# learningmatter-mit/surface-sampling

Hardware: AMD Instinct MI355X
Metric: MC energy-evaluations/sec (SrTiO3(001) ~250-atom slabs, 3-model PaiNN ensemble E+F incl. neighbor list) (higher is better)
Workload: dtype f32 via fp16x2-split MFMA (3 products), fp32 accumulate; neighbor decisions f64; 1 GPU; SrTiO3(001) PaiNN x3, 256 batched independent chains per GPU (BASELINE configs[3]), 248-272 atoms/chain; chains_per_gpu=256, atoms_per_gpu=66503, edges_per_gpu=2747786, slots_per_gpu=2836316, models=3, streams_per_gpu=2, parallelism=one GPU, no collective

## Files before the change

### surface-sampling_amd/csrc/api_batch.hip

```cpp
#include <cmath>
#include <cstdio>

#include "cell_dev.h"
#include "ewald_dev.h"

using namespace vssr;

extern "C" {

int vssr_batch_upload(vssr_handle *h, int32_t n_cfg, const int32_t *n_atoms, const int32_t *Z, const double *pos,
                      const double *cell, const uint8_t *pbc) {
    if (int rc = check_kind(h, KINDS_EVAL, __func__)) return rc;
    if (n_cfg < 1 || !n_atoms || !Z || !pos || !cell || !pbc) return set_err(h, VSSR_E_BADARG, "null or empty batch");
    VSSR_HIP(h, hipSetDevice(h->device));
    VSSR_HIP(h, hipStreamSynchronize(h->stream));
    h->batch_valid = false;
    h->ran = false;
    h->md_vel_valid = false;
    std::vector<int> start(n_cfg + 1, 0);
    for (int b = 0; b < n_cfg; ++b) {
        if (n_atoms[b] < 1) return set_err(h, VSSR_E_BADARG, "configuration %d has %d atoms", b, n_atoms[b]);
        if ((int64_t)start[b] + n_atoms[b] > 2000000000LL) return set_err(h, VSSR_E_BADARG, "batch too large");
        start[b + 1] = start[b] + n_atoms[b];
    }
// ... 571 lines not shown
    int l;
    if ((l = layer_of("phi")) >= 0) {
        if (l == 0 && h->l0_used)
            return set_err(h, VSSR_E_STATE, "phi0 is not materialised (layer-0 species factorisation is active)");
        src = sv.phi[l]; per_atom = F3;
    }
    else if ((l = layer_of("s_msg")) >= 0) { src = sv.s_msg[l]; per_atom = F; }
    else if ((l = layer_of("v_msg")) >= 0) { src = sv.v_msg[l]; per_atom = F3; }
    else if ((l = layer_of("s_upd")) >= 0) { src = sv.s_in[l + 1]; per_atom = F; }
    else if ((l = layer_of("v_upd")) >= 0) {
        if (l == h->num_conv - 1 && !h->debug_keep)
            return set_err(h, VSSR_E_STATE, "v_upd of the last block is not materialised (nothing consumes it; create the handle with VSSR_DEBUG_KEEP=1)");
        src = sv.v_in[l + 1]; per_atom = F3;
    }
    else if (nm == "e_atom") { src = sv.e_atom; per_atom = 1; }
    else if (nm == "sbar_msg0") { src = sv.sbar_msg_l0; per_atom = F; }
    else if (nm == "vbar_msg0") { src = sv.vbar_msg; per_atom = F3; }
    else return set_err(h, VSSR_E_BADARG, "unknown intermediate '%s'", name);
    size_t n = N * per_atom;
    *n_out = (int64_t)n;
    if (!dst) return VSSR_OK;
    if ((int64_t)n > cap) return set_err(h, VSSR_E_BADARG, "buffer too small for '%s'", name);
    VSSR_HIP(h, hipMemcpy(dst, src + (size_t)model * n, n * sizeof(float), hipMemcpyDeviceToHost));
    return VSSR_OK;
}

}
```

### surface-sampling_amd/csrc/api_painn.hip

```cpp
#include <cmath>

#include "vssr_internal.h"

namespace vssr {

static void transpose(const float *src, int rows, int cols, float *dst) {
    for (int r = 0; r < rows; ++r)
        for (int c = 0; c < cols; ++c) dst[(size_t)c * rows + r] = src[(size_t)r * cols + c];
}

static int upload_weights(vssr_handle *h, const vssr_painn_config *cfg) {
    const int M = cfg->n_models, L = cfg->num_conv, R = cfg->n_rbf, H = cfg->readout_hidden, NE = cfg->n_embed;
    const size_t per_layer = (size_t)F * F + F + (size_t)F3 * F + F3 + (size_t)F3 * R + F3 + 2 * (size_t)F * F +
                             (size_t)F * 2 * F + F + (size_t)F3 * F + F3;
    const size_t blob_len = (size_t)NE * F + L * per_layer + (size_t)H * F + H + H + 1;
    if (cfg->weights_len != blob_len)
        return set_err(h, VSSR_E_BADARG, "weights_len %llu does not match the layout (%zu floats)",
                       (unsigned long long)cfg->weights_len, blob_len);
    const size_t t_per_layer = (size_t)F * F + (size_t)F * F3 + 2 * (size_t)F * F + (size_t)2 * F * F + (size_t)F * F3;
    const size_t img_len = blob_len + L * t_per_layer + (size_t)F * H;
    std::vector<float> img(img_len * M);
    std::vector<ModelW> table(M);
    if (h->weights.ensure(img.size() * sizeof(float)))
        return set_err(h, VSSR_E_NOMEM, "weights: out of device memory");
// ... 115 lines not shown
        if (h->d_l0A.ensure(A16.size() * sizeof(unsigned)) || h->d_l0At.ensure(At16.size() * sizeof(unsigned)))
            return set_err(h, VSSR_E_NOMEM, "layer-0 tables");
        VSSR_HIP(h, hipMemcpy(h->d_l0A.p, A16.data(), A16.size() * sizeof(unsigned), hipMemcpyHostToDevice));
        VSSR_HIP(h, hipMemcpy(h->d_l0At.p, At16.data(), At16.size() * sizeof(unsigned), hipMemcpyHostToDevice));
    }
    if (h->model_table.ensure(sizeof(ModelW) * M)) return set_err(h, VSSR_E_NOMEM, "model table");
    VSSR_HIP(h, hipMemcpy(h->model_table.p, table.data(), sizeof(ModelW) * M, hipMemcpyHostToDevice));
    return VSSR_OK;
}

static void read_env_knobs(vssr_handle *h) {
    if (const char *e = getenv("VSSR_PAINN_PATH")) h->painn_general = h->painn_general || strcmp(e, "general") == 0;
    if (const char *e = getenv("VSSR_EDGE_IMPL")) h->edge_impl = (strcmp(e, "gather") == 0) ? 0 : 1;
    if (const char *e = getenv("VSSR_L0_FACTORISE")) h->l0_enabled = atoi(e);
    if (h->painn_general) h->l0_enabled = 0;
    if (const char *e = getenv("VSSR_UPD_SAVE")) h->upd_save = atoi(e);
    if (const char *e = getenv("VSSR_DEBUG_KEEP")) h->debug_keep = atoi(e);
    if (const char *e = getenv("VSSR_EDGE_FS16_MAX")) h->fs16_max_atoms = atoi(e);
    if (const char *e = getenv("VSSR_EDGE_FS8_MAX")) h->fs8_max_atoms = atoi(e);
    if (const char *e = getenv("VSSR_EDGE_BWD_MPASS")) h->bwd_multi_pass = atoi(e);
    if (const char *e = getenv("VSSR_EDGE_SUB_CHUNK")) { const int c = atoi(e); if (c >= 8) { h->sub_chunk_fwd = c; h->sub_chunk_bwd = c; } }
    if (const char *e = getenv("VSSR_EDGE_FWD_2PASS")) { const int w = atoi(e); h->fwd_two_pass = (w == 8 || w == 16) ? w : w ? 16 : 0; }
    if (const char *e = getenv("VSSR_EDGE_FWD_GRID")) h->edge_fwd_grid = max(atoi(e), 0);
}

}

using namespace vssr;

extern "C" {
// ... 47 lines not shown
```

### surface-sampling_amd/csrc/mfma16.h

```cpp
#ifndef VSSR_MFMA16_H
#define VSSR_MFMA16_H
#include "vssr_internal.h"

namespace vssr {

typedef float f32x4 __attribute__((ext_vector_type(4)));
typedef float f32x2 __attribute__((ext_vector_type(2)));
typedef unsigned u32x4 __attribute__((ext_vector_type(4)));
typedef unsigned u32x2 __attribute__((ext_vector_type(2)));
typedef _Float16 f16x8 __attribute__((ext_vector_type(8)));
typedef _Float16 f16x2 __attribute__((ext_vector_type(2)));

constexpr int TA = 32;
constexpr int NW = 8;
constexpr int NTHREADS = 64 * NW;
constexpr int PADH = 8;

#ifndef VSSR_FAST_SIGMOID
#define VSSR_FAST_SIGMOID 1
#endif
__device__ __forceinline__ float sigm(float x) {
#if VSSR_FAST_SIGMOID && defined(__HIP_DEVICE_COMPILE__)
    constexpr float C_HI = -1.44269502162933349609375f;
    constexpr float C_LO = -1.9259629911266175e-08f;
// ... 179 lines not shown
    return *reinterpret_cast<gptr>(reinterpret_cast<uintptr_t>(p));
#else
    return *reinterpret_cast<const f32x4 *>(p);
#endif
}

__device__ __forceinline__ float gload1f(const float *p) {
#if defined(__HIP_DEVICE_COMPILE__)
    typedef const float __attribute__((address_space(1))) *gptr;
    return *reinterpret_cast<gptr>(reinterpret_cast<uintptr_t>(p));
#else
    return *p;
#endif
}

}
#endif
```

### surface-sampling_amd/csrc/painn.hip

```cpp
#include "vssr_internal.h"

namespace vssr {

constexpr int T = NODE_TILE;
constexpr int RB = 21;
constexpr int ECHUNK = 16;
constexpr float PI_F = 3.14159265358979323846f;

__device__ inline float sigmoidf_(float x) { return 1.f / (1.f + expf(-x)); }
__device__ inline float swishf_(float x) { return x * sigmoidf_(x); }
__device__ inline float dswishf_(float x) {
    float sg = sigmoidf_(x);
    return sg * fmaf(x, 1.f - sg, 1.f);
}

__global__ void __launch_bounds__(128) k_embed(int N, const int *__restrict__ Z, const ModelW *__restrict__ MW,
                                               float *__restrict__ s0, float *__restrict__ v0) {
    int i = blockIdx.x, m = blockIdx.y, f = threadIdx.x;
    const ModelW &W = MW[m];
    size_t a = (size_t)m * N + i;
    s0[a * F + f] = W.embed[(size_t)Z[i] * F + f];
    v0[(a * 3 + 0) * F + f] = 0.f;
    v0[(a * 3 + 1) * F + f] = 0.f;
    v0[(a * 3 + 2) * F + f] = 0.f;
// ... 598 lines not shown
                launch_edge_fwd_mfma(st, cls, N, cls_list[cls], h->n_class[cls], M, l, h->max_class_atoms[cls], MW, G, counters,
                                     (int)(h->slot_cap - 1), sv.s_in[l], sv.v_in[l], sv.phi[l], sv.s_msg[l], sv.v_msg[l],
                                     (cls == EDGE_CLASS_FS4 && h->fwd_two_pass) ? h->d_bundle_sub.as<int4>() : (const int4 *)nullptr,
                                     h->fwd_two_pass, h->sub_chunk_fwd ? h->sub_chunk_fwd : sub_chunk_max(h->fwd_two_pass), h->edge_fwd_grid);
            if (n_gather)
                hipLaunchKernelGGL(k_edge_fwd<false>, g_atom, blk, 0, st, N, l, MW, G, counters, h->cutoff, h->excl_vol,
                                   h->excl_sigma, h->excl_power, sv.s_in[l], sv.v_in[l], sv.phi[l], sv.s_msg[l],
                                   sv.v_msg[l], (int)EDGE_BCLASS_GATHER);
        }
        P.end(st);
        update_fwd(l);
    }
    const bool fused = readout_mfma_supported(H);
    const bool want_forces = (want & VSSR_WANT_FORCES) != 0;
    const float *e_excl = h->excl_vol ? sv.e_excl : (const float *)nullptr;
    if (!(fused && want_forces)) {
        P.begin(KC_READOUT, st);
        if (fused) launch_readout_mfma(st, N, M, av, MW, sv.s_in[L], e_excl, sv.e_atom);
        else
            hipLaunchKernelGGL(k_readout, g_tile, blk, 0, st, N, H, av, MW, sv.s_in[L], sv.e_excl, h->excl_vol, sv.e_atom,
                               sv.sbar);
        P.end(st);
    }

    if (want_forces) {
        float *sb_buf[2] = {sv.sbar_msg, sv.sbar};
        for (int l = L - 1; l >= 0; --l) {
            float *sbar_msg_l = fused ? sb_buf[(L - 1 - l) & 1] : sv.sbar_msg;
            const float *sbar_msg_up = sb_buf[(L - l) & 1];
            P.begin(KC_UPDATE_BWD, st);
            if (!fused)
                launch_update_bwd_mfma(st, N, M, l, 0, (int)(l == L - 1), av, MW, sv.s_msg[l], sv.v_msg[l], sv.sbar, sv.vbar,
                                       nullptr, nullptr, nullptr, nullptr, sbar_msg_l, sv.vbar_msg, nullptr, nullptr);
            else if (l == L - 1 && fuse_last)
                launch_update_bwd_mfma(st, N, M, l, 3, 1, av, MW, sv.s_msg[l], sv.v_msg[l], nullptr, sv.vbar, nullptr, nullptr,
                                       e_excl, sv.e_atom, sbar_msg_l, sv.vbar_msg, sv.s_in[L], nullptr);
            else if (l == L - 1)
                launch_update_bwd_mfma(st, N, M, l, 1, 1, av, MW, sv.s_msg[l], sv.v_msg[l], nullptr, sv.vbar, sv.s_in[L], nullptr,
                                       e_excl, sv.e_atom, sbar_msg_l, sv.vbar_msg, nullptr, save_of(l));
            else
                launch_update_bwd_mfma(st, N, M, l, 2, 0, av, MW, sv.s_msg[l], sv.v_msg[l], sbar_msg_up, sv.vbar, sv.s_in[l + 1],
                                       sv.phibar, nullptr, nullptr, sbar_msg_l, sv.vbar_msg, nullptr, save_of(l));
            P.end(st);
            sv.sbar_msg_l0 = sbar_msg_l;
            P.begin((l == 0 && l0_fact) ? KC_L0_BWD : KC_EDGE_BWD, st);
            int accumulate = (l != L - 1);
            if (l == 0 && l0_fact) {
                rc = l0_run_reverse(h, G, (int)(L == 1), (int)partial, sbar_msg_l, sv.vbar_msg, sv.gbar);
                if (rc) return rc;
            } else if (l == 0)
                hipLaunchKernelGGL(k_edge_bwd<true>, g_atom, blk, 0, st, N, l, accumulate, MW, G, counters,
                                   h->cutoff, h->excl_vol, h->excl_sigma, h->excl_power, sv.v_in[l], sv.phi[l],
                                   sbar_msg_l, sv.vbar_msg, sv.phibar, sv.vbar, sv.gbar,
                                   (long long)h->slot_cap, -1, (int)partial);
            else {
                for (int cls = 0; cls < EDGE_MFMA_BCLASSES; ++cls)
                    launch_edge_bwd_mfma(st, cls, N, bcls_list[cls], h->n_bclass[cls], M, l, h->max_bclass_atoms[cls], MW, G, counters,
                                         (int)(h->slot_cap - 1), sv.v_in[l], sv.phi[l], sbar_msg_l, sv.vbar_msg, sv.phibar, sv.vbar,
                                         h->d_gpart.as<float>(), (long long)h->slot_cap, n_groups, (L - 1 - l) * per_set,
                                         cls == EDGE_BCLASS_FS16P ? h->d_bundle_subb.as<int4>() : (const int4 *)nullptr,
                                         h->sub_chunk_bwd ? h->sub_chunk_bwd : sub_chunk_max_bwd());
                if (n_gather)
                    hipLaunchKernelGGL(k_edge_bwd<false>, g_atom, blk, 0, st, N, l, accumulate, MW, G, counters,
// ... 11 lines not shown
    }
    P.begin(KC_FINALIZE, st);
    if (want_forces && partial) {
        const int uni = h->active_mask ? 0 : h->n_bclass[EDGE_BCLASS_FS16] + h->n_bclass[EDGE_BCLASS_FS16P] == h->n_cfg ? 8 : h->n_bclass[EDGE_BCLASS_FS8] == h->n_cfg ? 16
                        : h->n_bclass[EDGE_BCLASS_FS4] == h->n_cfg ? 32 : 0;
        const dim3 grid = uni ? dim3((unsigned)((h->slot_cap + 255) / 256), 1) : dim3(h->n_cfg, 12);
        hipLaunchKernelGGL(k_reduce_gpart, grid, dim3(256), 0, st, M, n_groups, layer_sets, G, counters, h->d_gpart.as<float>(),
                           sv.gbar, (long long)h->slot_cap, uni);
    }
    painn_finalize(h, G, want);
    P.end(st);
    VSSR_HIP(h, hipGetLastError());
    return VSSR_OK;
}

void painn_finalize(vssr_handle *h, const GraphView &G, uint32_t want) {
    const int N = h->n_atoms, M = h->n_models;
    hipStream_t st = h->stream;
    if (want & VSSR_WANT_FORCES)
        hipLaunchKernelGGL(k_finalize_forces, dim3((N + 3) / 4), dim3(256), 0, st, N, M, G, h->d_counters.as<int>(), h->sv.gbar,
                           (long long)h->slot_cap, h->units_per_ev, h->d_forces.as<float>(), h->d_forces_std.as<float>());
    hipLaunchKernelGGL(k_finalize_energy, dim3(h->n_cfg), dim3(256), 0, st, N, M, h->active_mask, G.cfg_start, h->d_Z.as<int>(),
                       h->sv.e_atom, h->units_per_ev, h->has_offset ? h->offset_per_z.as<double>() : (const double *)nullptr,
                       h->offset_const, h->d_energy.as<float>(), h->d_energy_std.as<float>(), h->d_energy_models.as<float>(),
                       h->d_energy64.as<double>(), h->d_e_atoms.as<float>(), h->d_sat.as<unsigned>(), h->d_sat_out.as<unsigned>());
}

int painn_stress(vssr_handle *h) {
    if (h->d_stress.ensure(sizeof(double) * 12 * (size_t)h->n_cfg)) return set_err(h, VSSR_E_DEVICE, "out of device memory (stress)");
    double *out = h->d_stress.as<double>();
// ... 8 lines not shown
```

### surface-sampling_amd/csrc/painn_l0.hip

```cpp
#include "mfma16.h"

namespace vssr {

constexpr int KP = 24;
constexpr int TBLK = 4 * KP;

template <int NZ>
__global__ void __launch_bounds__(96)
k_l0_accum(GraphView G, const int *__restrict__ counters, float *__restrict__ T) {
    constexpr int nz = NZ;
    if (counters[2] || !G.act.atom(blockIdx.x)) return;
    const int i = blockIdx.x, comp = threadIdx.x / KP, kap = threadIdx.x % KP;
    float acc[NZ];
#pragma unroll
    for (int z = 0; z < NZ; ++z) acc[z] = 0.f;
    auto erec_c = [&](int idx) -> float4 {
#if defined(__HIP_DEVICE_COMPILE__)
        typedef const f32x4 __attribute__((address_space(4))) *cp;
        const f32x4 v = reinterpret_cast<cp>(reinterpret_cast<uintptr_t>(G.erec))[idx];
        return make_float4(v.x, v.y, v.z, v.w);
#else
        return G.erec[idx];
#endif
    };
// ... 17 lines not shown
            r[u] = G.rho[(size_t)(e + u) * KP + kap];
            zi[u] = (zw >> (8 * u)) & 255;
        }
#pragma unroll
        for (int u = 0; u < 4; ++u) {
            const float uu = comp == 0 ? 1.f : comp == 1 ? er[u].x : comp == 2 ? er[u].y : er[u].z;
            const float val = r[u] * uu;
#pragma unroll
            for (int z = 0; z < NZ; ++z) acc[z] += (z == zi[u]) ? val : 0.f;
        }
    }
#pragma unroll
    for (int z = 0; z < NZ; ++z) T[((size_t)i * nz + z) * TBLK + comp * KP + kap] = acc[z];
}

constexpr int L0_TILE_U4 = 1024;

__global__ void __launch_bounds__(NTHREADS)
k_l0_fwd16(int N, int M, int nz, ActiveView av, const int *__restrict__ counters, const int *__restrict__ Z,
           const int *__restrict__ zlist, const ModelW *__restrict__ MW, const uint4 *__restrict__ A16, int n_embed,
           const float *__restrict__ T, float *__restrict__ s_msg, float *__restrict__ v_msg) {
    extern __shared__ __attribute__((aligned(16))) _Float16 ldsh[];
    if (counters[2]) return;
    const int K = 32 * nz, a0 = blockIdx.x * TA;
    if (!av.tile(min(a0, N - 1), min(a0 + TA - 1, N - 1))) return;
    const Planes Ts = make_planes(ldsh, TA, K), Tv = make_planes(ldsh + plane_halves(TA, K), 3 * TA, K);
    const LaneGeo L;
    SatTrack sat;
    const int lane = threadIdx.x & 63, r = lane & 15, g = lane >> 4;
    for (int t = threadIdx.x; t < TA * nz * 4 * 8; t += NTHREADS) {
        const int k4 = t & 7, comp = (t >> 3) & 3, z = (t >> 5) % nz, a = t / (32 * nz);
// ... 63 lines not shown
         float *__restrict__ Q ) {
    extern __shared__ __attribute__((aligned(16))) _Float16 ldsh[];
    if (counters[2]) return;
    const int a0 = blockIdx.x * TA, m = blockIdx.y;
    if (!av.tile(min(a0, N - 1), min(a0 + TA - 1, N - 1))) return;
    const size_t mN = (size_t)m * N;
    const Planes Xs = make_planes(ldsh, TA, F), Xv = make_planes(ldsh + plane_halves(TA, F), 3 * TA, F);
    SatTrack sat;
    load_rows_split<TA>(Xs, 0, [&](int row) { return sbar_msg + (mN + min(a0 + row, N - 1)) * F; }, sat);
    load_rows_split<3 * TA>(Xv, 0, [&](int row) {
        int x = row / TA, a = min(a0 + (row % TA), N - 1);
        return vbar_msg + ((mN + a) * 3 + x) * F;
    }, sat);
    sat.commit(av, a0, N);
    __syncthreads();
    const int lane = threadIdx.x & 63, r = lane & 15, g = lane >> 4, w = threadIdx.x >> 6;
    for (int ct = w; ct < 2 * nz; ct += NW) {
        const int q = ct >> 1, hf = ct & 1;
        const uint4 *wb = At16 + (((size_t)m * n_embed + zlist[q]) * 2) * L0_TILE_U4 + (size_t)hf * 512 + lane;
        f32x4 acc[8];
#pragma unroll
        for (int t = 0; t < 8; ++t) acc[t] = (f32x4){0.f, 0.f, 0.f, 0.f};
        u32x4 bb[2][2][2];
        auto load_w = [&](int buf, int c) {
#pragma unroll
            for (int sec = 0; sec < 2; ++sec)
#pragma unroll
                for (int pc = 0; pc < 2; ++pc) bb[buf][sec][pc] = gload4u(wb + sec * L0_TILE_U4 + (c * 2 + pc) * 64);
        };
        load_w(0, 0);
#pragma unroll
        for (int c = 0; c < F / 32; ++c) {
            u32x4 (&b)[2][2] = bb[c & 1];
            u32x4 a[8][2];
            if (c + 1 < F / 32) load_w((c + 1) & 1, c + 1);
#pragma unroll
            for (int t = 0; t < 8; ++t) {
                const Planes &P = t < 2 ? Xs : Xv;
                const int row = (t < 2 ? 16 * t : 16 * (t - 2)) + r;
                a[t][0] = *reinterpret_cast<const u32x4 *>(P.h + row * P.ld + 32 * c + 8 * g);
                a[t][1] = *reinterpret_cast<const u32x4 *>(P.l + row * P.ld + 32 * c + 8 * g);
            }
            __builtin_amdgcn_sched_barrier(0);
#pragma unroll
            for (int k = 0; k < 3; ++k)
#pragma unroll
                for (int t = 0; t < 8; ++t) {
                    acc[t] = mfma16(a[t][k == 1 ? 1 : 0], b[t < 2 ? 0 : 1][k == 0 ? 1 : 0], acc[t]);
                    __builtin_amdgcn_sched_barrier(0);
                }
        }
        const int kap = 16 * hf + r;
        if (kap < KP) {
#pragma unroll
            for (int t = 0; t < 8; ++t) {
                const int comp = t < 2 ? 0 : 1 + (t - 2) / 2, tt = t < 2 ? t : (t - 2) & 1;
#pragma unroll
                for (int i = 0; i < 4; ++i) {
                    const int a_ = a0 + 16 * tt + 4 * g + i;
                    if (a_ < N) Q[((((size_t)m * N + a_) * nz + q) * 4 + comp) * KP + kap] = acc[t][i];
                }
            }
        }
    }
}

__global__ void __launch_bounds__(256)
k_l0_bwd(int N, int M, int nz, int first_write, int fresh_mfma, int excl_vol, float rc, GraphView G, const int *__restrict__ counters,
         const float *__restrict__ Q, float4 *__restrict__ gbar, long long slot_cap) {
    extern __shared__ __attribute__((aligned(16))) float qs_all[];
    const int lane = threadIdx.x & 63, wave = threadIdx.x >> 6, sl = lane >> 2, kq = lane & 3;
    const int n = blockIdx.x * (blockDim.x >> 6) + wave;
    if (n >= N || counters[2] || !G.act.atom(n)) return;
    const int per_model = nz * TBLK;
    const bool fw = first_write || (fresh_mfma && G.chain_class[G.atom_cfg[n]] != EDGE_BCLASS_GATHER);
    float *qs = qs_all + (size_t)wave * M * per_model;
    for (int m = 0; m < M; ++m) {
        const float4 *src = reinterpret_cast<const float4 *>(Q + ((size_t)m * N + n) * per_model);
        for (int i = lane; i < per_model / 4; i += 64) reinterpret_cast<float4 *>(qs + m * per_model)[i] = src[i];
// ... 135 lines not shown
            default: hipLaunchKernelGGL(k_l0_accum<L0_MAX_SPECIES>, dim3(N), dim3(96), 0, st, G, cnt, T); break;
        }
    }
    const size_t lds_fwd = sizeof(_Float16) * (plane_halves(TA, 32 * nz) + plane_halves(3 * TA, 32 * nz));
    hipLaunchKernelGGL(k_l0_fwd16, dim3((N + TA - 1) / TA), dim3(NTHREADS), lds_fwd, st, N, M, nz, G.act, h->d_counters.as<int>(),
                       h->d_Z.as<int>(), h->d_zlist.as<int>(), h->model_table.as<ModelW>(), h->d_l0A.as<uint4>(), h->n_embed,
                       h->d_l0T.as<float>(), s_msg, v_msg);
    return VSSR_OK;
}

int l0_run_reverse(vssr_handle *h, const GraphView &G, int first_write, int fresh_mfma, const float *sbar_msg, const float *vbar_msg,
                   float4 *gbar) {
    const int N = h->n_atoms, M = h->n_models, nz = h->l0_nz;
    hipStream_t st = h->stream;
    const size_t lds_q = sizeof(_Float16) * (plane_halves(TA, F) + plane_halves(3 * TA, F));
    hipLaunchKernelGGL(k_l0_q16, dim3((N + TA - 1) / TA, M), dim3(NTHREADS), lds_q, st, N, nz, G.act, h->d_counters.as<int>(),
                       h->d_zlist.as<int>(), h->d_l0At.as<uint4>(), h->n_embed, sbar_msg, vbar_msg, h->d_l0Q.as<float>());
    if (sizeof(float) * 4 * M * nz * TBLK > 48 * 1024)
        VSSR_HIP(h, hipFuncSetAttribute((const void *)k_l0_bwd, hipFuncAttributeMaxDynamicSharedMemorySize, 160 * 1024));
    hipLaunchKernelGGL(k_l0_bwd, dim3((N + 3) / 4), dim3(256), sizeof(float) * 4 * M * nz * TBLK, st, N, M, nz, first_write, fresh_mfma,
                       h->excl_vol, h->cutoff, G, h->d_counters.as<int>(), h->d_l0Q.as<float>(), gbar, (long long)h->slot_cap);
    return VSSR_OK;
}

}
```

### surface-sampling_amd/csrc/painn_node_mfma.hip

```cpp
#include "mfma16.h"

#ifdef PHASE_TIMING
__device__ unsigned long long g_phase[64];
#define PH_INIT unsigned long long ph_t = wall_clock64();
#define PH_RESET ph_t = wall_clock64();
#define PH(k) { const unsigned long long ph_n = wall_clock64(); if (threadIdx.x == 0) atomicAdd(&g_phase[k], ph_n - ph_t); ph_t = wall_clock64(); }
extern "C" int vssr_debug_phases(unsigned long long *out, int reset) {
    if (hipMemcpyFromSymbol(out, HIP_SYMBOL(g_phase), sizeof(unsigned long long) * 64) != hipSuccess) return -1;
    if (reset) { unsigned long long z[64] = {}; if (hipMemcpyToSymbol(HIP_SYMBOL(g_phase), z, sizeof(z)) != hipSuccess) return -1; }
    return 0;
}
#else
#define PH_INIT
#define PH_RESET
#define PH(k)
#endif

namespace vssr {

template <int NRT, int NCT>
struct GemmShape {
    static constexpr int NT = NRT * NCT, NACC = NT >= 3 ? 1 : 2;
};
template <int NRT, int NCT, int NPRE>
// ... 691 lines not shown
    extern __shared__ __attribute__((aligned(16))) _Float16 ldsh[];
    const int m = blockIdx.y, a0 = blockIdx.x * TA;
    if (!av.tile(min(a0, N - 1), min(a0 + TA - 1, N - 1))) return;
    const LaneGeo L;
    SatTrack sat;
    const size_t mN = (size_t)m * N;
    const Planes xs = make_planes(ldsh, TA, F), hp = make_planes(ldsh + plane_halves(TA, F), TA, RH);
    float *red = reinterpret_cast<float *>(ldsh + plane_halves(TA, F) + plane_halves(TA, RH));
    load_rows_split<TA>(xs, 0, [&](int row) { return s + (mN + min(a0 + row, N - 1)) * F; }, sat);
    __syncthreads();
    f32x4 sb[2];
    readout_head<2, false>(MW[m], xs, hp, red, L, a0, N, mN, e_excl, e_atom, sb, sat);
    sat.commit(av, a0, N);
}

template <int MODE, int RT, bool SAVED = false>
__global__ void __launch_bounds__(NTHREADS) __attribute__((amdgpu_waves_per_eu(RT == 1 ? 4 : 2, RT == 1 ? 4 : 2)))
k_update_bwd_mfma(int N, int l, int vbar_is_zero, ActiveView av, const ModelW *__restrict__ MW, const float *__restrict__ s_msg,
                  const float *__restrict__ v_msg, const float *__restrict__ sbar_src, const float *__restrict__ vbar,
                  const float *__restrict__ s_next, const float *__restrict__ phibar, const float *__restrict__ e_excl,
                  float *__restrict__ e_atom, float *__restrict__ sbar_msg, float *__restrict__ vbar_msg,
                  float *__restrict__ s_last, const f32x4 *__restrict__ save) {
    static_assert(!SAVED || RT == 2, "the saved layout is that of the 32-atom forward kernel");
    constexpr bool FUSED = MODE == 3;
    static_assert(!FUSED || (!SAVED && RT == 2), "the fused last block runs its own forward pass on 32-atom tiles");
    static_assert(MODE != 1 || SAVED, "without stored intermediates the last layer is MODE 3");
    extern __shared__ __attribute__((aligned(16))) _Float16 ldsh[];
    constexpr int TA = 16 * RT, OFF_VT = UpdLds<RT>::OFF_VT, OFF_AS = UpdLds<RT>::OFF_AS, UPD_LDS_HALVES = UpdLds<RT>::HALVES;
    const int m = blockIdx.y, a0 = blockIdx.x * TA;
    if (!av.tile(min(a0, N - 1), min(a0 + TA - 1, N - 1))) return;
    const LaneGeo L;
    constexpr int BPF = MODE == 0 ? 0 : UPD_PF;
    SatNone unwatched;
    const LayerW &W = MW[m].layer[l];
    const size_t mN = (size_t)m * N;
    PH_INIT
    f32x4 sb[RT];
    if (MODE != 1 && !FUSED) {
// ... 246 lines not shown
        const uint4 *wp[1] = {WTILE(UVt, L.w, 2 * F)};
        gemm16<2 * F, 3 * RT, 1, BPF>(ab, wp, out);
    }
    PH(31)
    __syncthreads();
    PH(32)
    float *T = reinterpret_cast<float *>(ldsh);
#pragma unroll
    for (int t = 0; t < RT; ++t) {
        const int row = L.row(t);
        *reinterpret_cast<f32x4 *>(T + row * FT + L.col0) = sb[t] + hbar[t][0];
#pragma unroll
        for (int x = 0; x < 3; ++x) *reinterpret_cast<f32x4 *>(T + (TA * (1 + x) + row) * FT + L.col0) = out[RT * x + t][0];
    }
    __syncthreads();
    stage_rows<4 * TA>(T, [&](int row, int col, const float4 &d) {
        const int q = row / TA, a = a0 + row % TA;
        if (a >= N) return;
        if (q == 0) {
            *reinterpret_cast<float4 *>(sbar_msg + (mN + a) * F + col) = d;
        } else {
            const size_t off = ((mN + a) * 3 + (q - 1)) * F + col;
            float4 r = make_float4(0.f, 0.f, 0.f, 0.f);
            if (!vbar_is_zero) r = *reinterpret_cast<const float4 *>(VB + (row - TA) * FT + col);
            *reinterpret_cast<float4 *>(vbar_msg + off) = make_float4(r.x + d.x, r.y + d.y, r.z + d.z, r.w + d.w);
        }
    });
    PH(33)
}

// ... 44 lines not shown
    VSSR_HIP(h, hipFuncSetAttribute((const void *)k_update_fwd_mfma<0>, hipFuncAttributeMaxDynamicSharedMemorySize,
                                    (int)node_mfma_lds_bytes(6)));
    VSSR_HIP(h, hipFuncSetAttribute((const void *)k_update_fwd_mfma<1>, hipFuncAttributeMaxDynamicSharedMemorySize,
                                    (int)node_mfma_lds_bytes(6)));
    VSSR_HIP(h, hipFuncSetAttribute((const void *)k_update_fwd_mfma<2>, hipFuncAttributeMaxDynamicSharedMemorySize,
                                    (int)node_mfma_lds_bytes(6)));
#define SET_UPD(MODE)                                                                                                     \
    VSSR_HIP(h, hipFuncSetAttribute((const void *)k_update_bwd_mfma<MODE, 2>, hipFuncAttributeMaxDynamicSharedMemorySize, \
                                    (int)node_mfma_lds_bytes(3)));
    SET_UPD(0) SET_UPD(2) SET_UPD(3)
#undef SET_UPD
    VSSR_HIP(h, hipFuncSetAttribute((const void *)k_update_bwd_mfma<1, 2, true>, hipFuncAttributeMaxDynamicSharedMemorySize,
                                    (int)node_mfma_lds_bytes(3)));
    VSSR_HIP(h, hipFuncSetAttribute((const void *)k_update_bwd_mfma<2, 2, true>, hipFuncAttributeMaxDynamicSharedMemorySize,
                                    (int)node_mfma_lds_bytes(3)));
    VSSR_HIP(h, hipFuncSetAttribute((const void *)k_readout_mfma, hipFuncAttributeMaxDynamicSharedMemorySize,
                                    (int)node_mfma_lds_bytes(4)));
    return VSSR_OK;
}

void launch_msg_mlp_mfma(hipStream_t st, int N, int M, int l, const ActiveView &av, const ModelW *MW, const float *s_in,
                         float *phi) {
    hipLaunchKernelGGL((k_msg_mlp_mfma<2, 0>), dim3((N + TA - 1) / TA, M), dim3(NTHREADS), node_mfma_lds_bytes(0), st, N, l, av, MW,
                       s_in, phi);
}
void launch_msg_mlp_bwd_mfma(hipStream_t st, int N, int M, int l, const ActiveView &av, const ModelW *MW, const float *s_in,
                             const float *phibar, const float *sbar_msg, float *sbar_in) {
    hipLaunchKernelGGL(k_msg_mlp_bwd_mfma, dim3((N + TA - 1) / TA, M), dim3(NTHREADS), node_mfma_lds_bytes(1), st, N, l, av, MW,
                       s_in, phibar, sbar_msg, sbar_in);
}
// ... 6 lines not shown
    else if (!v_out && !sv)
        hipLaunchKernelGGL(k_update_fwd_mfma<2>, dim3((N + TA - 1) / TA, M), dim3(NTHREADS), node_mfma_lds_bytes(6), st, N, l,
                           av, MW, s_msg, v_msg, s_out, v_out, phi_next, sv);
    else
        hipLaunchKernelGGL(k_update_fwd_mfma<0>, dim3((N + TA - 1) / TA, M), dim3(NTHREADS), node_mfma_lds_bytes(6), st, N, l,
                           av, MW, s_msg, v_msg, s_out, v_out, phi_next, sv);
}
void launch_readout_mfma(hipStream_t st, int N, int M, const ActiveView &av, const ModelW *MW, const float *s,
                         const float *e_excl, float *e_atom) {
    hipLaunchKernelGGL(k_readout_mfma, dim3((N + TA - 1) / TA, M), dim3(NTHREADS), node_mfma_lds_bytes(4), st, N, av, MW, s,
                       e_excl, e_atom);
}
void launch_update_bwd_mfma(hipStream_t st, int N, int M, int l, int mode, int vbar_is_zero, const ActiveView &av, const ModelW *MW,
                            const float *s_msg, const float *v_msg, const float *sbar_src, const float *vbar,
                            const float *s_next, const float *phibar, const float *e_excl, float *e_atom,
                            float *sbar_msg, float *vbar_msg, float *s_last, const void *save) {
    const f32x4 *sv = reinterpret_cast<const f32x4 *>(save);
    if (mode == 1 || mode == 3) vbar_is_zero = 1;
#if defined(UPD_BWD_RT) && UPD_BWD_RT == 1
    if (!sv && mode == 2) {
        const dim3 grid1((N + 15) / 16, M), blk1(NTHREADS);
        const size_t lds1 = sizeof(_Float16) * UpdLds<1>::HALVES + sizeof(float) * 3 * 16 * FT;
        static bool once = [] {
            (void)hipFuncSetAttribute((const void *)k_update_bwd_mfma<2, 1, false>, hipFuncAttributeMaxDynamicSharedMemorySize, 80 * 1024);
            return true;
        }();
        (void)once;
        hipLaunchKernelGGL((k_update_bwd_mfma<2, 1, false>), grid1, blk1, lds1, st, N, l, vbar_is_zero, av, MW, s_msg, v_msg, sbar_src,
                           vbar, s_next, phibar, e_excl, e_atom, sbar_msg, vbar_msg, s_last, sv);
        return;
    }
#endif
    const dim3 grid((N + TA - 1) / TA, M), blk(NTHREADS);
    const size_t lds = node_mfma_lds_bytes(3);
#define LAUNCH_UPD(MODE, SAVED)                                                                                             \
    hipLaunchKernelGGL((k_update_bwd_mfma<MODE, 2, SAVED>), grid, blk, lds, st, N, l, vbar_is_zero, av, MW, s_msg, v_msg, sbar_src, \
                       vbar, s_next, phibar, e_excl, e_atom, sbar_msg, vbar_msg, s_last, sv)
    if (mode == 1) LAUNCH_UPD(1, true);
    else if (mode == 2) { if (sv) LAUNCH_UPD(2, true); else LAUNCH_UPD(2, false); }
    else if (mode == 3) LAUNCH_UPD(3, false);
    else LAUNCH_UPD(0, false);
#undef LAUNCH_UPD
}

}
```

### surface-sampling_amd/csrc/vssr_internal.h

```cpp
#pragma once

#include <hip/hip_runtime.h>

#include <cstdint>
#include <cstdio>
#include <cstdlib>
#include <cstring>
#include <initializer_list>
#include <memory>
#include <string>
#include <type_traits>
#include <utility>
#include <vector>

#include "../../include/vssr_eval.h"

namespace vssr {

constexpr int F = 128;
constexpr int F3 = 3 * F;
constexpr int MAX_LAYERS = 4;
constexpr int MAX_MODELS = 8;
constexpr int RB_MAX = 24;
constexpr int NODE_TILE = 8;
// ... 307 lines not shown
    bool batch_valid = false, ran = false;
    int n_cfg = 0, n_atoms = 0;
    std::vector<int> h_n_atoms, h_cfg_start;
    vssr::DevBuf d_pos, d_wpos, d_wrap, d_Z, d_atom_cfg, d_cfg_start, d_cell, d_invcell, d_nimg, d_pbc;
    vssr::DevBuf d_deg, d_row_start, d_edge, d_edge_S, d_rev, d_counters, d_tile_sums;
    vssr::DevBuf d_erec, d_rho, d_dist, d_rho16, d_drho16, d_zslot, d_bundle, d_excl;
    vssr::DevBuf d_bundle_sub;
    int bwd_multi_pass = 1;
    int sub_chunk_fwd = 0, sub_chunk_bwd = 0;
    vssr::DevBuf d_bundle_subb;
    int fwd_two_pass = 16;
    int edge_fwd_grid = -1;
    vssr::DevBuf d_hits;
    int l0_enabled = 1, l0_nz = 0;
    bool l0_used = false;
    vssr::DevBuf d_l0A, d_l0At;
    vssr::DevBuf d_zmap, d_zlist;
    vssr::DevBuf d_l0T, d_l0Q;
    vssr::DevBuf d_opt_state, d_opt_vec, d_bfgs_q, d_bfgs_b, d_fixed, d_relax_steps, d_relax_conv, d_active;
    const unsigned char *active_mask = nullptr;
    int relax_regrows = 0;
    long long relax_lockstep = 0;
    int relax_compactions = 0;
    vssr::DevBuf d_cmp;
    vssr::DevBuf d_cm;
    long long relax_chain_evals = 0;
    int traj_interval = 0, traj_records = 0, traj_B = 0, traj_N = 0;
    vssr::DevBuf d_traj_pos, d_traj_f, d_traj_e, d_traj_n;
    bool graph_partial = false;
    bool l0T_by_geom = false;
// ... 149 lines not shown
int relax_cg(vssr_handle *h, const vssr_cg_params *cp, const uint8_t *fixed_host, uint32_t want);
int relax_bfgsls(vssr_handle *h, const vssr_bfgsls_params *bp, const uint8_t *fixed_host, uint32_t want);
bool chain_min_supported(const vssr_handle *h);
int chain_min_cg(vssr_handle *h, const vssr_cg_params *cp, const uint8_t *fixed_host, uint32_t want);
int node_mfma_init(vssr_handle *h);
void launch_msg_mlp_mfma(hipStream_t st, int N, int M, int l, const ActiveView &av, const ModelW *MW, const float *s_in,
                         float *phi);
void launch_msg_mlp_bwd_mfma(hipStream_t st, int N, int M, int l, const ActiveView &av, const ModelW *MW, const float *s_in,
                             const float *phibar, const float *sbar_msg, float *sbar_in);
void launch_update_fwd_mfma(hipStream_t st, int N, int M, int l, const ActiveView &av, const ModelW *MW, const float *s_msg,
                            const float *v_msg, float *s_out, float *v_out, float *phi_next, void *save);
size_t update_save_bytes(int N, int M);
bool readout_mfma_supported(int hidden);
void launch_readout_mfma(hipStream_t st, int N, int M, const ActiveView &av, const ModelW *MW, const float *s, const float *e_excl,
                         float *e_atom);
void launch_update_bwd_mfma(hipStream_t st, int N, int M, int l, int mode, int vbar_is_zero, const ActiveView &av, const ModelW *MW,
                            const float *s_msg, const float *v_msg, const float *sbar_src, const float *vbar,
                            const float *s_next, const float *phibar, const float *e_excl, float *e_atom,
                            float *sbar_msg, float *vbar_msg, float *s_last, const void *save);
void pack_mfma_tiles16(const float *Wsrc, int rows, int K, unsigned *dst );
void build_wd16(const float *Wd, const float *bd, unsigned *dst );
void l0_build_tables(const float *blob_embed, const float *W1, const float *b1, const float *W2, const float *b2,
                     const float *Wd, const float *bd, int n_embed, float *A, float *At);
void l0_pack_tables(const float *A, int n_embed, unsigned *A16, unsigned *At16);
size_t l0_packed_dwords(int n_embed);
int l0_mfma_init(vssr_handle *h);
int l0_run_forward(vssr_handle *h, const GraphView &G, float *s_msg, float *v_msg);
int l0_run_reverse(vssr_handle *h, const GraphView &G, int first_write, int fresh_mfma, const float *sbar_msg, const float *vbar_msg,
                   float4 *gbar);
int edge_mfma_init(vssr_handle *h);
enum { EDGE_CLASS_FS16 = 0, EDGE_CLASS_FS16M = 1, EDGE_CLASS_FS8 = 2, EDGE_CLASS_FS4 = 3, EDGE_CLASS_GATHER = 4, EDGE_CLASSES = 5,
       EDGE_MFMA_CLASSES = 4 };
enum { EDGE_BCLASS_FS16 = 0, EDGE_BCLASS_FS8 = 1, EDGE_BCLASS_FS4 = 2, EDGE_BCLASS_FS16P = 3, EDGE_BCLASS_GATHER = 4, EDGE_BCLASSES = 5,
       EDGE_MFMA_BCLASSES = 4 };
__host__ __device__ constexpr int edge_bclass_slices(int c) { return (c == EDGE_BCLASS_FS16 || c == EDGE_BCLASS_FS16P) ? 8 : c == EDGE_BCLASS_FS8 ? 16 : c == EDGE_BCLASS_FS4 ? 32 : 1; }
int edge_bclass_of(int n_atoms);
int edge_class_of(int n_atoms);
constexpr int SUB_MAX_PASSES = 4;
__host__ __device__ constexpr int sub_chunk_max(int width) { return width == 16 ? 400 : 784; }
__host__ __device__ constexpr int sub_chunk_max_bwd() { return 550; }
__host__ __device__ constexpr int sub_passes(int n_atoms, int chunk_max) { return (n_atoms + chunk_max - 1) / chunk_max; }
__host__ __device__ constexpr int sub_chunk(int n_atoms, int chunk_max) { return (n_atoms + sub_passes(n_atoms, chunk_max) - 1) / sub_passes(n_atoms, chunk_max); }
int edge_class_groups(int cls);
void launch_edge_bwd_mfma(hipStream_t st, int cls, int N, const int *list, int n_list, int M, int l, int max_atoms,
// ... 11 lines not shown
```

Measured before the change: 25220 evaluations/s.

## Fuse layer-0 Q contraction into the layer-0 update backward kernel

Moves the layer-0 factorised Q contraction (previously a separate k_l0_q16 launch that reread sbar_msg/vbar_msg from global memory) into the tail of the mode-2 update-backward kernel. The adjoint tiles are split into fp16 planes directly in LDS and contracted there, which skips writing sbar_msg_l0/vbar_msg to global memory and one kernel launch. For debug reads of those intermediates, a helper recomputes them on demand. The fused kernel gains extra LDS work and register pressure, and the path is bypassed when upd_save is set.

Result: no change. 25170 evaluations/s (-0.2%).

```diff
diff --git a/surface-sampling_amd/csrc/api_batch.hip b/surface-sampling_amd/csrc/api_batch.hip
--- a/surface-sampling_amd/csrc/api_batch.hip
+++ b/surface-sampling_amd/csrc/api_batch.hip
@@ -609,8 +609,11 @@
         src = sv.v_in[l + 1]; per_atom = F3;
     }
     else if (nm == "e_atom") { src = sv.e_atom; per_atom = 1; }
-    else if (nm == "sbar_msg0") { src = sv.sbar_msg_l0; per_atom = F; }
-    else if (nm == "vbar_msg0") { src = sv.vbar_msg; per_atom = F3; }
+    else if (nm == "sbar_msg0" || nm == "vbar_msg0") {
+        if (dst && (rc = painn_debug_l0_adjoints(h))) return rc;
+        if (nm == "sbar_msg0") { src = sv.sbar_msg_l0; per_atom = F; }
+        else { src = sv.vbar_msg; per_atom = F3; }
+    }
     else return set_err(h, VSSR_E_BADARG, "unknown intermediate '%s'", name);
     size_t n = N * per_atom;
     *n_out = (int64_t)n;
diff --git a/surface-sampling_amd/csrc/api_painn.hip b/surface-sampling_amd/csrc/api_painn.hip
--- a/surface-sampling_amd/csrc/api_painn.hip
+++ b/surface-sampling_amd/csrc/api_painn.hip
@@ -153,6 +153,7 @@
     if (const char *e = getenv("VSSR_EDGE_IMPL")) h->edge_impl = (strcmp(e, "gather") == 0) ? 0 : 1;
     if (const char *e = getenv("VSSR_L0_FACTORISE")) h->l0_enabled = atoi(e);
     if (h->painn_general) h->l0_enabled = 0;
+    if (const char *e = getenv("VSSR_L0_FUSE")) h->l0_fuse = atoi(e);
     if (const char *e = getenv("VSSR_UPD_SAVE")) h->upd_save = atoi(e);
     if (const char *e = getenv("VSSR_DEBUG_KEEP")) h->debug_keep = atoi(e);
     if (const char *e = getenv("VSSR_EDGE_FS16_MAX")) h->fs16_max_atoms = atoi(e);
diff --git a/surface-sampling_amd/csrc/mfma16.h b/surface-sampling_amd/csrc/mfma16.h
--- a/surface-sampling_amd/csrc/mfma16.h
+++ b/surface-sampling_amd/csrc/mfma16.h
@@ -217,5 +217,63 @@
 #endif
 }
 
-}
-#endif
+constexpr int KP = 24;
+constexpr int TBLK = 4 * KP;
+constexpr int L0_TILE_U4 = 1024;
+
+__device__ __forceinline__ void l0_q_contract(int tid, const Planes &Xs, const Planes &Xv, int N, int nz, int m, int a0,
+                                              const int *__restrict__ zlist, const uint4 *__restrict__ At16, int n_embed,
+                                              float *__restrict__ Q ) {
+    const int lane = tid & 63, r = lane & 15, g = lane >> 4, w = tid >> 6;
+    for (int ct = w; ct < 2 * nz; ct += NW) {
+        const int q = ct >> 1, hf = ct & 1;
+        const uint4 *wb = At16 + (((size_t)m * n_embed + zlist[q]) * 2) * L0_TILE_U4 + (size_t)hf * 512 + lane;
+        f32x4 acc[8];
+#pragma unroll
+        for (int t = 0; t < 8; ++t) acc[t] = (f32x4){0.f, 0.f, 0.f, 0.f};
+        u32x4 bb[2][2][2];
+        auto load_w = [&](int buf, int c) {
+#pragma unroll
+            for (int sec = 0; sec < 2; ++sec)
+#pragma unroll
+                for (int pc = 0; pc < 2; ++pc) bb[buf][sec][pc] = gload4u(wb + sec * L0_TILE_U4 + (c * 2 + pc) * 64);
+        };
+        load_w(0, 0);
+#pragma unroll
+        for (int c = 0; c < F / 32; ++c) {
+            u32x4 (&b)[2][2] = bb[c & 1];
+            u32x4 a[8][2];
+            if (c + 1 < F / 32) load_w((c + 1) & 1, c + 1);
+#pragma unroll
+            for (int t = 0; t < 8; ++t) {
+                const Planes &P = t < 2 ? Xs : Xv;
+                const int row = (t < 2 ? 16 * t : 16 * (t - 2)) + r;
+                a[t][0] = *reinterpret_cast<const u32x4 *>(P.h + row * P.ld + 32 * c + 8 * g);
+                a[t][1] = *reinterpret_cast<const u32x4 *>(P.l + row * P.ld + 32 * c + 8 * g);
+            }
+            __builtin_amdgcn_sched_barrier(0);
+#pragma unroll
+            for (int k = 0; k < 3; ++k)
+#pragma unroll
+                for (int t = 0; t < 8; ++t) {
+                    acc[t] = mfma16(a[t][k == 1 ? 1 : 0], b[t < 2 ? 0 : 1][k == 0 ? 1 : 0], acc[t]);
+                    __builtin_amdgcn_sched_barrier(0);
+                }
+        }
+        const int kap = 16 * hf + r;
+        if (kap < KP) {
+#pragma unroll
+            for (int t = 0; t < 8; ++t) {
+                const int comp = t < 2 ? 0 : 1 + (t - 2) / 2, tt = t < 2 ? t : (t - 2) & 1;
+#pragma unroll
+                for (int i = 0; i < 4; ++i) {
+                    const int a_ = a0 + 16 * tt + 4 * g + i;
+                    if (a_ < N) Q[((((size_t)m * N + a_) * nz + q) * 4 + comp) * KP + kap] = acc[t][i];
+                }
+            }
+        }
+    }
+}
+
+}
+#endif
diff --git a/surface-sampling_amd/csrc/painn.hip b/surface-sampling_amd/csrc/painn.hip
--- a/surface-sampling_amd/csrc/painn.hip
+++ b/surface-sampling_amd/csrc/painn.hip
@@ -636,6 +636,8 @@
     const bool fused = readout_mfma_supported(H);
     const bool want_forces = (want & VSSR_WANT_FORCES) != 0;
     const float *e_excl = h->excl_vol ? sv.e_excl : (const float *)nullptr;
+    const bool l0_q_fused = l0_fact && h->l0_fuse && fused && L >= 2 && !h->upd_save;
+    h->l0_adj_fused = false;
     if (!(fused && want_forces)) {
         P.begin(KC_READOUT, st);
         if (fused) launch_readout_mfma(st, N, M, av, MW, sv.s_in[L], e_excl, sv.e_atom);
@@ -660,7 +662,13 @@
             else if (l == L - 1)
                 launch_update_bwd_mfma(st, N, M, l, 1, 1, av, MW, sv.s_msg[l], sv.v_msg[l], nullptr, sv.vbar, sv.s_in[L], nullptr,
                                        e_excl, sv.e_atom, sbar_msg_l, sv.vbar_msg, nullptr, save_of(l));
-            else
+            else if (l == 0 && l0_q_fused) {
+                const L0QTail q0 = l0_q_tail(h);
+                launch_update_bwd_mfma(st, N, M, l, 2, 0, av, MW, sv.s_msg[l], sv.v_msg[l], sbar_msg_up, sv.vbar, sv.s_in[l + 1],
+                                       sv.phibar, nullptr, nullptr, sbar_msg_l, sv.vbar_msg, nullptr, nullptr, &q0);
+                h->l0_adj_fused = true;
+                h->l0_sbar_up = sbar_msg_up;
+            } else
                 launch_update_bwd_mfma(st, N, M, l, 2, 0, av, MW, sv.s_msg[l], sv.v_msg[l], sbar_msg_up, sv.vbar, sv.s_in[l + 1],
                                        sv.phibar, nullptr, nullptr, sbar_msg_l, sv.vbar_msg, nullptr, save_of(l));
             P.end(st);
@@ -668,7 +676,7 @@
             P.begin((l == 0 && l0_fact) ? KC_L0_BWD : KC_EDGE_BWD, st);
             int accumulate = (l != L - 1);
             if (l == 0 && l0_fact) {
-                rc = l0_run_reverse(h, G, (int)(L == 1), (int)partial, sbar_msg_l, sv.vbar_msg, sv.gbar);
+                rc = l0_run_reverse(h, G, (int)(L == 1), (int)partial, l0_q_fused ? nullptr : sbar_msg_l, sv.vbar_msg, sv.gbar);
                 if (rc) return rc;
             } else if (l == 0)
                 hipLaunchKernelGGL(k_edge_bwd<true>, g_atom, blk, 0, st, N, l, accumulate, MW, G, counters,
@@ -710,6 +718,19 @@
     return VSSR_OK;
 }
 
+int painn_debug_l0_adjoints(vssr_handle *h) {
+    if (!h->l0_adj_fused) return VSSR_OK;
+    const StateView &sv = h->sv;
+    ActiveView av = graph_view(h).act;
+    av.sat = nullptr;
+    launch_update_bwd_mfma(h->stream, h->n_atoms, h->n_models, 0, 2, 0, av, h->model_table.as<ModelW>(), sv.s_msg[0], sv.v_msg[0],
+                           h->l0_sbar_up, sv.vbar, sv.s_in[1], sv.phibar, nullptr, nullptr, sv.sbar_msg_l0, sv.vbar_msg, nullptr, nullptr);
+    VSSR_HIP(h, hipGetLastError());
+    VSSR_HIP(h, hipStreamSynchronize(h->stream));
+    h->l0_adj_fused = false;
+    return VSSR_OK;
+}
+
 void painn_finalize(vssr_handle *h, const GraphView &G, uint32_t want) {
     const int N = h->n_atoms, M = h->n_models;
     hipStream_t st = h->stream;
diff --git a/surface-sampling_amd/csrc/painn_l0.hip b/surface-sampling_amd/csrc/painn_l0.hip
--- a/surface-sampling_amd/csrc/painn_l0.hip
+++ b/surface-sampling_amd/csrc/painn_l0.hip
@@ -2,8 +2,6 @@
 
 namespace vssr {
 
-constexpr int KP = 24;
-constexpr int TBLK = 4 * KP;
 
 template <int NZ>
 __global__ void __launch_bounds__(96)
@@ -55,7 +53,6 @@
     for (int z = 0; z < NZ; ++z) T[((size_t)i * nz + z) * TBLK + comp * KP + kap] = acc[z];
 }
 
-constexpr int L0_TILE_U4 = 1024;
 
 __global__ void __launch_bounds__(NTHREADS)
 k_l0_fwd16(int N, int M, int nz, ActiveView av, const int *__restrict__ counters, const int *__restrict__ Z,
@@ -149,55 +146,7 @@
     }, sat);
     sat.commit(av, a0, N);
     __syncthreads();
-    const int lane = threadIdx.x & 63, r = lane & 15, g = lane >> 4, w = threadIdx.x >> 6;
-    for (int ct = w; ct < 2 * nz; ct += NW) {
-        const int q = ct >> 1, hf = ct & 1;
-        const uint4 *wb = At16 + (((size_t)m * n_embed + zlist[q]) * 2) * L0_TILE_U4 + (size_t)hf * 512 + lane;
-        f32x4 acc[8];
-#pragma unroll
-        for (int t = 0; t < 8; ++t) acc[t] = (f32x4){0.f, 0.f, 0.f, 0.f};
-        u32x4 bb[2][2][2];
-        auto load_w = [&](int buf, int c) {
-#pragma unroll
-            for (int sec = 0; sec < 2; ++sec)
-#pragma unroll
-                for (int pc = 0; pc < 2; ++pc) bb[buf][sec][pc] = gload4u(wb + sec * L0_TILE_U4 + (c * 2 + pc) * 64);
-        };
-        load_w(0, 0);
-#pragma unroll
-        for (int c = 0; c < F / 32; ++c) {
-            u32x4 (&b)[2][2] = bb[c & 1];
-            u32x4 a[8][2];
-            if (c + 1 < F / 32) load_w((c + 1) & 1, c + 1);
-#pragma unroll
-            for (int t = 0; t < 8; ++t) {
-                const Planes &P = t < 2 ? Xs : Xv;
-                const int row = (t < 2 ? 16 * t : 16 * (t - 2)) + r;
-                a[t][0] = *reinterpret_cast<const u32x4 *>(P.h + row * P.ld + 32 * c + 8 * g);
-                a[t][1] = *reinterpret_cast<const u32x4 *>(P.l + row * P.ld + 32 * c + 8 * g);
-            }
-            __builtin_amdgcn_sched_barrier(0);
-#pragma unroll
-            for (int k = 0; k < 3; ++k)
-#pragma unroll
-                for (int t = 0; t < 8; ++t) {
-                    acc[t] = mfma16(a[t][k == 1 ? 1 : 0], b[t < 2 ? 0 : 1][k == 0 ? 1 : 0], acc[t]);
-                    __builtin_amdgcn_sched_barrier(0);
-                }
-        }
-        const int kap = 16 * hf + r;
-        if (kap < KP) {
-#pragma unroll
-            for (int t = 0; t < 8; ++t) {
-                const int comp = t < 2 ? 0 : 1 + (t - 2) / 2, tt = t < 2 ? t : (t - 2) & 1;
-#pragma unroll
-                for (int i = 0; i < 4; ++i) {
-                    const int a_ = a0 + 16 * tt + 4 * g + i;
-                    if (a_ < N) Q[((((size_t)m * N + a_) * nz + q) * 4 + comp) * KP + kap] = acc[t][i];
-                }
-            }
-        }
-    }
+    l0_q_contract(threadIdx.x, Xs, Xv, N, nz, m, a0, zlist, At16, n_embed, Q);
 }
 
 __global__ void __launch_bounds__(256)
@@ -363,8 +312,9 @@
     const int N = h->n_atoms, M = h->n_models, nz = h->l0_nz;
     hipStream_t st = h->stream;
     const size_t lds_q = sizeof(_Float16) * (plane_halves(TA, F) + plane_halves(3 * TA, F));
-    hipLaunchKernelGGL(k_l0_q16, dim3((N + TA - 1) / TA, M), dim3(NTHREADS), lds_q, st, N, nz, G.act, h->d_counters.as<int>(),
-                       h->d_zlist.as<int>(), h->d_l0At.as<uint4>(), h->n_embed, sbar_msg, vbar_msg, h->d_l0Q.as<float>());
+    if (sbar_msg)
+        hipLaunchKernelGGL(k_l0_q16, dim3((N + TA - 1) / TA, M), dim3(NTHREADS), lds_q, st, N, nz, G.act, h->d_counters.as<int>(),
+                           h->d_zlist.as<int>(), h->d_l0At.as<uint4>(), h->n_embed, sbar_msg, vbar_msg, h->d_l0Q.as<float>());
     if (sizeof(float) * 4 * M * nz * TBLK > 48 * 1024)
         VSSR_HIP(h, hipFuncSetAttribute((const void *)k_l0_bwd, hipFuncAttributeMaxDynamicSharedMemorySize, 160 * 1024));
     hipLaunchKernelGGL(k_l0_bwd, dim3((N + 3) / 4), dim3(256), sizeof(float) * 4 * M * nz * TBLK, st, N, M, nz, first_write, fresh_mfma,
@@ -372,4 +322,8 @@
     return VSSR_OK;
 }
 
-}
+L0QTail l0_q_tail(const vssr_handle *h) {
+    return L0QTail{h->d_counters.as<int>(), h->d_zlist.as<int>(), h->d_l0At.as<uint4>(), h->d_l0Q.as<float>(), h->l0_nz, h->n_embed};
+}
+
+}
diff --git a/surface-sampling_amd/csrc/painn_node_mfma.hip b/surface-sampling_amd/csrc/painn_node_mfma.hip
--- a/surface-sampling_amd/csrc/painn_node_mfma.hip
+++ b/surface-sampling_amd/csrc/painn_node_mfma.hip
@@ -729,14 +729,15 @@
     sat.commit(av, a0, N);
 }
 
-template <int MODE, int RT, bool SAVED = false>
+template <int MODE, int RT, bool SAVED = false, bool L0Q = false>
 __global__ void __launch_bounds__(NTHREADS) __attribute__((amdgpu_waves_per_eu(RT == 1 ? 4 : 2, RT == 1 ? 4 : 2)))
 k_update_bwd_mfma(int N, int l, int vbar_is_zero, ActiveView av, const ModelW *__restrict__ MW, const float *__restrict__ s_msg,
                   const float *__restrict__ v_msg, const float *__restrict__ sbar_src, const float *__restrict__ vbar,
                   const float *__restrict__ s_next, const float *__restrict__ phibar, const float *__restrict__ e_excl,
                   float *__restrict__ e_atom, float *__restrict__ sbar_msg, float *__restrict__ vbar_msg,
-                  float *__restrict__ s_last, const f32x4 *__restrict__ save) {
+                  float *__restrict__ s_last, const f32x4 *__restrict__ save, L0QTail q0) {
     static_assert(!SAVED || RT == 2, "the saved layout is that of the 32-atom forward kernel");
+    static_assert(!L0Q || (MODE == 2 && RT == 2 && !SAVED), "the layer-0 contraction rides on the 32-atom mode-2 kernel");
     constexpr bool FUSED = MODE == 3;
     static_assert(!FUSED || (!SAVED && RT == 2), "the fused last block runs its own forward pass on 32-atom tiles");
     static_assert(MODE != 1 || SAVED, "without stored intermediates the last layer is MODE 3");
@@ -1013,6 +1014,38 @@
         for (int x = 0; x < 3; ++x) *reinterpret_cast<f32x4 *>(T + (TA * (1 + x) + row) * FT + L.col0) = out[RT * x + t][0];
     }
     __syncthreads();
+    if constexpr (L0Q) {
+        constexpr int NIT = 4 * TA * (F / 4) / NTHREADS, NS = TA * (F / 4) / NTHREADS;
+        static_assert(plane_halves(TA, F) + plane_halves(3 * TA, F) <= UPD_LDS_HALVES, "Q planes end in front of the vbar tile");
+        int tid = threadIdx.x;
+        asm volatile("" : "+v"(tid));
+        tid &= NTHREADS - 1;
+        float4 val[NIT];
+#pragma unroll
+        for (int it = 0; it < NIT; ++it) {
+            const int idx = tid + it * NTHREADS, row = idx >> 5, c4 = idx & 31;
+            const float4 d = *reinterpret_cast<const float4 *>(T + row * FT + 4 * c4);
+            if (it < NS) { val[it] = d; continue; }
+            float4 r = make_float4(0.f, 0.f, 0.f, 0.f);
+            if (!vbar_is_zero) r = *reinterpret_cast<const float4 *>(VB + (row - TA) * FT + 4 * c4);
+            val[it] = make_float4(r.x + d.x, r.y + d.y, r.z + d.z, r.w + d.w);
+        }
+        __syncthreads();
+        const Planes Xs = make_planes(ldsh, TA, F), Xv = make_planes(ldsh + plane_halves(TA, F), 3 * TA, F);
+        SatTrack satq;
+#pragma unroll
+        for (int it = 0; it < NIT; ++it) {
+            const int idx = tid + it * NTHREADS, row = idx >> 5, c4 = idx & 31;
+            if (it < NS) store_split4<SAT_COOP>(Xs, row, 4 * c4, val[it], satq);
+            else store_split4<SAT_COOP>(Xv, row - TA, 4 * c4, val[it], satq);
+        }
+        satq.commit(av, a0, N);
+        __syncthreads();
+        PH(33)
+        if (!q0.counters[2]) l0_q_contract(tid, Xs, Xv, N, q0.nz, m, a0, q0.zlist, q0.At16, q0.n_embed, q0.Q);
+        PH(34)
+        return;
+    }
     stage_rows<4 * TA>(T, [&](int row, int col, const float4 &d) {
         const int q = row / TA, a = a0 + row % TA;
         if (a >= N) return;
@@ -1087,6 +1120,8 @@
                                     (int)node_mfma_lds_bytes(3)));
     VSSR_HIP(h, hipFuncSetAttribute((const void *)k_update_bwd_mfma<2, 2, true>, hipFuncAttributeMaxDynamicSharedMemorySize,
                                     (int)node_mfma_lds_bytes(3)));
+    VSSR_HIP(h, hipFuncSetAttribute((const void *)k_update_bwd_mfma<2, 2, false, true>, hipFuncAttributeMaxDynamicSharedMemorySize,
+                                    (int)node_mfma_lds_bytes(3)));
     VSSR_HIP(h, hipFuncSetAttribute((const void *)k_readout_mfma, hipFuncAttributeMaxDynamicSharedMemorySize,
                                     (int)node_mfma_lds_bytes(4)));
     return VSSR_OK;
@@ -1123,8 +1158,9 @@
 void launch_update_bwd_mfma(hipStream_t st, int N, int M, int l, int mode, int vbar_is_zero, const ActiveView &av, const ModelW *MW,
                             const float *s_msg, const float *v_msg, const float *sbar_src, const float *vbar,
                             const float *s_next, const float *phibar, const float *e_excl, float *e_atom,
-                            float *sbar_msg, float *vbar_msg, float *s_last, const void *save) {
+                            float *sbar_msg, float *vbar_msg, float *s_last, const void *save, const L0QTail *q0) {
     const f32x4 *sv = reinterpret_cast<const f32x4 *>(save);
+    const L0QTail qt = q0 ? *q0 : L0QTail{nullptr, nullptr, nullptr, nullptr, 0, 0};
     if (mode == 1 || mode == 3) vbar_is_zero = 1;
 #if defined(UPD_BWD_RT) && UPD_BWD_RT == 1
     if (!sv && mode == 2) {
@@ -1136,19 +1172,19 @@
         }();
         (void)once;
         hipLaunchKernelGGL((k_update_bwd_mfma<2, 1, false>), grid1, blk1, lds1, st, N, l, vbar_is_zero, av, MW, s_msg, v_msg, sbar_src,
-                           vbar, s_next, phibar, e_excl, e_atom, sbar_msg, vbar_msg, s_last, sv);
+                           vbar, s_next, phibar, e_excl, e_atom, sbar_msg, vbar_msg, s_last, sv, qt);
         return;
     }
 #endif
     const dim3 grid((N + TA - 1) / TA, M), blk(NTHREADS);
     const size_t lds = node_mfma_lds_bytes(3);
-#define LAUNCH_UPD(MODE, SAVED)                                                                                             \
-    hipLaunchKernelGGL((k_update_bwd_mfma<MODE, 2, SAVED>), grid, blk, lds, st, N, l, vbar_is_zero, av, MW, s_msg, v_msg, sbar_src, \
-                       vbar, s_next, phibar, e_excl, e_atom, sbar_msg, vbar_msg, s_last, sv)
-    if (mode == 1) LAUNCH_UPD(1, true);
-    else if (mode == 2) { if (sv) LAUNCH_UPD(2, true); else LAUNCH_UPD(2, false); }
-    else if (mode == 3) LAUNCH_UPD(3, false);
-    else LAUNCH_UPD(0, false);
+#define LAUNCH_UPD(MODE, SAVED, L0Q)                                                                                        \
+    hipLaunchKernelGGL((k_update_bwd_mfma<MODE, 2, SAVED, L0Q>), grid, blk, lds, st, N, l, vbar_is_zero, av, MW, s_msg, v_msg, sbar_src, \
+                       vbar, s_next, phibar, e_excl, e_atom, sbar_msg, vbar_msg, s_last, sv, qt)
+    if (mode == 1) LAUNCH_UPD(1, true, false);
+    else if (mode == 2) { if (sv) LAUNCH_UPD(2, true, false); else if (qt.Q) LAUNCH_UPD(2, false, true); else LAUNCH_UPD(2, false, false); }
+    else if (mode == 3) LAUNCH_UPD(3, false, false);
+    else LAUNCH_UPD(0, false, false);
 #undef LAUNCH_UPD
 }
 
diff --git a/surface-sampling_amd/csrc/vssr_internal.h b/surface-sampling_amd/csrc/vssr_internal.h
--- a/surface-sampling_amd/csrc/vssr_internal.h
+++ b/surface-sampling_amd/csrc/vssr_internal.h
@@ -345,6 +345,9 @@
     vssr::DevBuf d_hits;
     int l0_enabled = 1, l0_nz = 0;
     bool l0_used = false;
+    int l0_fuse = 1;
+    bool l0_adj_fused = false;
+    const float *l0_sbar_up = nullptr;
     vssr::DevBuf d_l0A, d_l0At;
     vssr::DevBuf d_zmap, d_zlist;
     vssr::DevBuf d_l0T, d_l0Q;
@@ -524,10 +527,16 @@
 bool readout_mfma_supported(int hidden);
 void launch_readout_mfma(hipStream_t st, int N, int M, const ActiveView &av, const ModelW *MW, const float *s, const float *e_excl,
                          float *e_atom);
+struct L0QTail {
+    const int *counters, *zlist;
+    const uint4 *At16;
+    float *Q;
+    int nz, n_embed;
+};
 void launch_update_bwd_mfma(hipStream_t st, int N, int M, int l, int mode, int vbar_is_zero, const ActiveView &av, const ModelW *MW,
                             const float *s_msg, const float *v_msg, const float *sbar_src, const float *vbar,
                             const float *s_next, const float *phibar, const float *e_excl, float *e_atom,
-                            float *sbar_msg, float *vbar_msg, float *s_last, const void *save);
+                            float *sbar_msg, float *vbar_msg, float *s_last, const void *save, const L0QTail *q0 = nullptr);
 void pack_mfma_tiles16(const float *Wsrc, int rows, int K, unsigned *dst );
 void build_wd16(const float *Wd, const float *bd, unsigned *dst );
 void l0_build_tables(const float *blob_embed, const float *W1, const float *b1, const float *W2, const float *b2,
@@ -538,6 +547,8 @@
 int l0_run_forward(vssr_handle *h, const GraphView &G, float *s_msg, float *v_msg);
 int l0_run_reverse(vssr_handle *h, const GraphView &G, int first_write, int fresh_mfma, const float *sbar_msg, const float *vbar_msg,
                    float4 *gbar);
+L0QTail l0_q_tail(const vssr_handle *h);
+int painn_debug_l0_adjoints(vssr_handle *h);
 int edge_mfma_init(vssr_handle *h);
 enum { EDGE_CLASS_FS16 = 0, EDGE_CLASS_FS16M = 1, EDGE_CLASS_FS8 = 2, EDGE_CLASS_FS4 = 3, EDGE_CLASS_GATHER = 4, EDGE_CLASSES = 5,
        EDGE_MFMA_CLASSES = 4 };
```
